# gabrielfnayres/new-vit

Hardware: AMD Instinct MI355X
Metric: volumes_per_sec_mst_dinov2_fwd (higher is better)
Workload: dtype bf16; 1 GPU; MST-DINOv2 (DinoV2ClassifierSlice, ViT-S/14) forward, 4 volumes/GPU of 64x512x512 bf16 zero-padded to 518x518 (N=1370 tokens/slice); global_batch_volumes=4, slices=64, parallelism=single GPU, weights=synthetic (mst.synth seed 2), random init of the reference architecture

## Files before the change

### new-vit_amd/csrc/k_gemm16_wreg.hip

```cpp
#include <cstdlib>

#include "mst_common.h"

namespace {

constexpr int KD = GEMM16_WREG_TILE.bk, BN = GEMM16_WREG_TILE.bn, CH = GEMM16_WREG_TILE.bm;
constexpr int ROWB = KD * 2;
constexpr int SLOT = CH * ROWB;
constexpr int WREG_NSLOT = 4;
constexpr int NSLOT = WREG_NSLOT;
constexpr int STG_PITCH = ROWB + 16;
constexpr int STG_BYTES = CH * STG_PITCH;
constexpr int STG_OFF = NSLOT * SLOT;
constexpr int LDS_BYTES = STG_OFF + 2 * STG_BYTES;
constexpr int NKT = KD / 32;
constexpr int PPW = SLOT / 1024 / 8;
static_assert(NSLOT == 4, "the counted vmcnt table below is written for three chunks in flight");

#define WREG_RD(dst, base, imm) asm volatile("ds_read_b128 %0, %1 offset:%2" : "=v"(dst) : "v"(base), "n"(imm) : "memory")

template <typename T, bool BLK>
__global__ __launch_bounds__(512) __attribute__((amdgpu_waves_per_eu(2, 2))) void gemm16_wreg_kernel(
    const T* __restrict__ A, int64_t lda, const T* __restrict__ W, int64_t ldw, const float* __restrict__ bias, T* __restrict__ C,
    int64_t ldc, int M, int N, float col_scale, int scale_cols, int nchunks) {
    typedef typename V8<T>::type vec8;
    typedef __attribute__((ext_vector_type(4))) T out4;
    extern __shared__ __attribute__((aligned(16))) char smem[];
    const int lane = threadIdx.x & 63;
    const int wave = __builtin_amdgcn_readfirstlane(threadIdx.x >> 6);
    const int frow = lane & 15, kq = lane >> 4;

    const int xcd = blockIdx.x & 7, g = blockIdx.x >> 3, G = gridDim.x >> 3;
    const int tiles_n = N / BN;
    const int nt = g % tiles_n, jcu = g / tiles_n;
    const int c_nt = (G - nt + tiles_n - 1) / tiles_n;
    const int per_xcd = (nchunks + 7) >> 3;
    const int lo = xcd * per_xcd;
    const int hi = lo + per_xcd < nchunks ? lo + per_xcd : nchunks;
    const int n0 = nt * BN + wave * 48;
    const float cs = nt * BN < scale_cols ? col_scale : 1.f;

    vec8 w[3][NKT];
#pragma unroll
    for (int t = 0; t < 3; ++t) {
        const T* wr = W + (int64_t)(n0 + 12 * (frow >> 2) + 4 * t + (frow & 3)) * ldw + kq * 8;
#pragma unroll
        for (int kt = 0; kt < NKT; ++kt) w[t][kt] = *reinterpret_cast<const vec8*>(wr + kt * 32);
    }
    f32x4 b[3];
#pragma unroll
    for (int t = 0; t < 3; ++t) {
        b[t] = (f32x4){0.f, 0.f, 0.f, 0.f};
        if (bias) b[t] = *reinterpret_cast<const f32x4*>(bias + n0 + 12 * kq + 4 * t);
    }
#pragma unroll
    for (int t = 0; t < 3; ++t) {
        asm volatile("" : "+v"(b[t]));
#pragma unroll
        for (int kt = 0; kt < NKT; ++kt) asm volatile("" : "+v"(w[t][kt]));
    }

    unsigned dma_off[PPW];
#pragma unroll
    for (int u = 0; u < PPW; ++u) {
        const int o = (wave * PPW + u) * 1024 + lane * 16;
        const int r = o / ROWB;
        dma_off[u] = BLK ? (unsigned)o : (unsigned)(r * (int)lda * 2 + ((((o % ROWB) >> 4) ^ (r & 15)) << 4));
    }
    const int64_t chunk_bytes = BLK ? (int64_t)SLOT : (int64_t)CH * lda * 2;
    auto issue_piece = [&](int chunk, int slot, int u) {
        const char* base = reinterpret_cast<const char*>(A) + (int64_t)chunk * chunk_bytes;
        unsigned off = dma_off[u];
        const int valid = M - chunk * CH;
        if (!BLK && valid < CH) {
            const int o = (wave * PPW + u) * 1024 + lane * 16;
            int r = o / ROWB;
            const int ck = ((o % ROWB) >> 4) ^ (r & 15);
            r = r < valid ? r : valid - 1;
            off = (unsigned)(r * (int)lda * 2 + ck * 16);
        }
        __builtin_amdgcn_global_load_lds(GLB_PTR(base + off), LDS_PTR(smem + slot * SLOT + (wave * PPW + u) * 1024), 16, 0, 0);
    };

    int rb[4];
#pragma unroll
    for (int j = 0; j < 4; ++j) rb[j] = BLK ? (kq >> 1) * 1024 + (frow + 32 * (kq & 1)) * 16 : frow * ROWB + (((4 * j + kq) ^ frow) << 4);
    const int put_off = frow * STG_PITCH + wave * 96 + kq * 24;
    int fl_lds[3];
    unsigned fl_glb[3];
    int fl_row[3];
#pragma unroll
    for (int j = 0; j < 3; ++j) {
        const int q = lane + 64 * j;
        fl_row[j] = wave * 4 + q / 48;
        fl_lds[j] = fl_row[j] * STG_PITCH + (q % 48) * 16;
        fl_glb[j] = (unsigned)(fl_row[j] * (int)ldc * 2 + nt * BN * 2 + (q % 48) * 16);
    }
    f32x4 acc[2][3];
    auto put = [&](int it) {
        char* stg = smem + STG_OFF + (it & 1) * STG_BYTES + put_off;
#pragma unroll
        for (int mt = 0; mt < 2; ++mt)
#pragma unroll
            for (int t = 0; t < 3; ++t) {
                out4 pk;
#pragma unroll
                for (int i = 0; i < 4; ++i) pk[i] = (T)(acc[mt][t][i] * cs);
                *reinterpret_cast<out4*>(stg + mt * 16 * STG_PITCH + t * 8) = pk;
            }
    };
    auto flush_piece = [&](int chunk, int it, int j) {
        const char* stg = smem + STG_OFF + (it & 1) * STG_BYTES;
        char* cb = reinterpret_cast<char*>(C) + (int64_t)chunk * CH * ldc * 2;
        const int valid = M - chunk * CH;
        const u32x4 v = *reinterpret_cast<const u32x4*>(stg + fl_lds[j]);
        if (valid >= CH || fl_row[j] < valid) {
            __builtin_nontemporal_store(v, reinterpret_cast<u32x4*>(cb + fl_glb[j]));
        }
    };
    auto flush = [&](int chunk, int it) {
#pragma unroll
        for (int j = 0; j < 3; ++j) flush_piece(chunk, it, j);
    };

    int c = lo + jcu;
    if (c >= hi) return;
#pragma unroll
    for (int d = 0; d < NSLOT - 1; ++d)
        if (c + d * c_nt < hi) {
#pragma unroll
            for (int u = 0; u < PPW; ++u) issue_piece(c + d * c_nt, d, u);
        }

    int prev = -1, last_it = 0;
    for (int it = 0; c < hi; c += c_nt, ++it) {
        if (c + 2 * c_nt < hi) {
            if (it <= 1) asm volatile("s_waitcnt vmcnt(6)" ::: "memory");
            else if (it == 2) asm volatile("s_waitcnt vmcnt(9)" ::: "memory");
            else asm volatile("s_waitcnt vmcnt(12)" ::: "memory");
        } else {
            asm volatile("s_waitcnt vmcnt(0)" ::: "memory");
        }
        asm volatile("s_waitcnt lgkmcnt(0)\n\ts_barrier" ::: "memory");
        if (prev >= 0) flush(prev, it - 1);

        const int slot = it % NSLOT;
        const int nxt = c + (NSLOT - 1) * c_nt, nslot = (it + NSLOT - 1) % NSLOT;
        const bool more = nxt < hi;
        int rbs[4];
#pragma unroll
        for (int j = 0; j < 4; ++j) rbs[j] = rb[j] + slot * SLOT;
#pragma unroll
        for (int mt = 0; mt < 2; ++mt)
#pragma unroll
            for (int t = 0; t < 3; ++t) acc[mt][t] = b[t];

        u32x4 a[2][2];
        WREG_RD(a[0][0], rbs[0], 0);
        if constexpr (BLK) WREG_RD(a[0][1], rbs[0], 256);
        else WREG_RD(a[0][1], rbs[0], 16 * ROWB);
#pragma unroll
        for (int kt = 0; kt < NKT; ++kt) {
            const int cur = kt & 1;
            if (kt + 1 < NKT) {
                switch (kt + 1) {
#define WREG_NEXT(KN)                                                                  \
    case KN:                                                                           \
        if constexpr (BLK) {                                                           \
            WREG_RD(a[(KN) & 1][0], rbs[0], (KN) * 2048);                              \
            WREG_RD(a[(KN) & 1][1], rbs[0], (KN) * 2048 + 256);                        \
        } else {                                                                       \
            WREG_RD(a[(KN) & 1][0], rbs[(KN) & 3], ((KN) >> 2) * 256);                 \
            WREG_RD(a[(KN) & 1][1], rbs[(KN) & 3], 16 * ROWB + ((KN) >> 2) * 256);     \
        }                                                                              \
        break;
                    WREG_NEXT(1) WREG_NEXT(2) WREG_NEXT(3) WREG_NEXT(4) WREG_NEXT(5) WREG_NEXT(6)
                    WREG_NEXT(7) WREG_NEXT(8) WREG_NEXT(9) WREG_NEXT(10) WREG_NEXT(11)
#undef WREG_NEXT
                }
                asm volatile("s_waitcnt lgkmcnt(2)" : "+v"(a[cur][0]), "+v"(a[cur][1])::"memory");
            } else {
                asm volatile("s_waitcnt lgkmcnt(0)" : "+v"(a[cur][0]), "+v"(a[cur][1])::"memory");
            }
            const vec8 a0 = __builtin_bit_cast(vec8, a[cur][0]), a1 = __builtin_bit_cast(vec8, a[cur][1]);
#pragma unroll
            for (int t = 0; t < 3; ++t) {
                acc[0][t] = mfma16(w[t][kt], a0, acc[0][t]);
                acc[1][t] = mfma16(w[t][kt], a1, acc[1][t]);
            }
            if ((kt & 3) == 1) {
                __builtin_amdgcn_sched_barrier(0);
                if (more) issue_piece(nxt, nslot, kt >> 2);
                __builtin_amdgcn_sched_barrier(0);
            }
        }
        put(it);
        prev = c;
        last_it = it;
    }
    asm volatile("s_waitcnt lgkmcnt(0)\n\ts_barrier" ::: "memory");
    flush(prev, last_it);
}

template <typename T, bool BLK>
int launch_t(const gemm_args& g) {
    static mst_lds_once lds_once;
    auto kern = gemm16_wreg_kernel<T, BLK>;
    mst_allow_lds((const void*)kern, LDS_BYTES, &lds_once);
    const int nchunks = (int)((g.M + CH - 1) / CH);
    kern<<<dim3(mst_persistent_grid()), dim3(512), LDS_BYTES, g.s>>>((const T*)g.A, g.lda, (const T*)g.W, g.ldw, g.bias, (T*)g.C, g.ldc, (int)g.M,
                                                                      g.N, g.col_scale, g.scale_cols, nchunks);
    return mst_check_launch("gemm16_wreg");
}

}

int launch_gemm16_wreg(const gemm_args& g, int a_blocked) {
    if (a_blocked) {
        if (g.dt == MST_BF16) return launch_t<bf16_t, true>(g);
        if (g.dt == MST_F16) return launch_t<f16_t, true>(g);
    }
    if (g.dt == MST_BF16) return launch_t<bf16_t, false>(g);
    if (g.dt == MST_F16) return launch_t<f16_t, false>(g);
    mst_set_error("gemm16_wreg: bad operand dtype %d", g.dt);
    return MST_EINVAL;
}
```

Baseline: 161.2 volumes/s.

## Balance QKV GEMM tiles across CUs and overlap epilogue with MFMA loop

Replaces the fixed tile-per-workgroup assignment with a segment schedule. Leftover column tiles that do not divide evenly across workgroups are split into short runs handled by spare workgroups, which reload weights for each segment. The schedule is checked at compile time for coverage and per-workgroup load bounds. The epilogue is now software-pipelined: the previous chunk's results are staged to LDS, and the chunk before that is read back and stored to global memory, interleaved between MFMA steps instead of in a serialized phase after the barrier. This aims to cut tail imbalance and epilogue stalls, at the cost of more complex waitcnt accounting and extra weight reloads for spare workgroups.

```diff
diff --git a/new-vit_amd/csrc/k_gemm16_wreg.hip b/new-vit_amd/csrc/k_gemm16_wreg.hip
--- a/new-vit_amd/csrc/k_gemm16_wreg.hip
+++ b/new-vit_amd/csrc/k_gemm16_wreg.hip
@@ -19,6 +19,53 @@
 
 #define WREG_RD(dst, base, imm) asm volatile("ds_read_b128 %0, %1 offset:%2" : "=v"(dst) : "v"(base), "n"(imm) : "memory")
 
+constexpr int WREG_RELOAD_UNITS = 2;
+constexpr int wreg_spare_run(int G, int T, int P) {
+    const int S = G % T;
+    if (!S) return 0;
+    int n = (2 * P + G) / (2 * G);
+    const int allow = ((T - 1) * WREG_RELOAD_UNITS + T - 1) / T;
+    n -= allow < n / 8 ? allow : n / 8;
+    if (S * n > P) n = P / S;
+    const int teams = G / T, bound = (T * P + G - 1) / G + 1;
+    while ((P - S * n + teams - 1) / teams > bound && T * (n + 1) <= bound) ++n;
+    return n;
+}
+struct wreg_seg { int tile, first, step, end; };
+constexpr int wreg_nseg(int g, int G, int T) { return g < G / T * T ? 1 : T; }
+constexpr wreg_seg wreg_segment(int g, int G, int T, int P, int k) {
+    const int teams = G / T, n = wreg_spare_run(G, T, P);
+    if (g < teams * T) return {g % T, (G % T) * n + g / T, teams, P};
+    const int s = g - teams * T;
+    return {k, s * n, 1, (s + 1) * n};
+}
+constexpr bool wreg_sched_ok(int G, int T, int P) {
+    int seen[4 * 1370] = {};
+    if (T * P > 4 * 1370 || T > G) return false;
+    const int bound = (T * P + G - 1) / G + 1;
+    for (int g = 0; g < G; ++g) {
+        int units = 0;
+        for (int k = 0; k < wreg_nseg(g, G, T); ++k) {
+            const wreg_seg s = wreg_segment(g, G, T, P, k);
+            if (s.tile < 0 || s.tile >= T || s.first < 0 || s.step < 1 || s.end > P) return false;
+            for (int c = s.first; c < s.end; c += s.step, ++units) ++seen[s.tile * P + c];
+        }
+        if (units > bound) return false;
+    }
+    for (int u = 0; u < T * P; ++u)
+        if (seen[u] != 1) return false;
+    return true;
+}
+constexpr bool wreg_sched_ok_all(int G) {
+    constexpr int Ps[] = {0, 1, 2, 3, 10, 11, 12, 33, 49, 1370};
+    for (int T = 1; T <= 4; ++T)
+        for (int P : Ps)
+            if (!wreg_sched_ok(G, T, P)) return false;
+    return true;
+}
+static_assert(wreg_sched_ok_all(32), "QKV schedule: a unit is missed or doubled, or a workgroup is over ceil(T P / G) + 1 (MI355X, 32 CUs per XCD)");
+static_assert(wreg_sched_ok_all(4) && wreg_sched_ok_all(5) && wreg_sched_ok_all(7), "QKV schedule at other CU counts per XCD");
+
 template <typename T, bool BLK>
 __global__ __launch_bounds__(512) __attribute__((amdgpu_waves_per_eu(2, 2))) void gemm16_wreg_kernel(
     const T* __restrict__ A, int64_t lda, const T* __restrict__ W, int64_t ldw, const float* __restrict__ bias, T* __restrict__ C,
@@ -32,33 +79,10 @@
 
     const int xcd = blockIdx.x & 7, g = blockIdx.x >> 3, G = gridDim.x >> 3;
     const int tiles_n = N / BN;
-    const int nt = g % tiles_n, jcu = g / tiles_n;
-    const int c_nt = (G - nt + tiles_n - 1) / tiles_n;
     const int per_xcd = (nchunks + 7) >> 3;
     const int lo = xcd * per_xcd;
-    const int hi = lo + per_xcd < nchunks ? lo + per_xcd : nchunks;
-    const int n0 = nt * BN + wave * 48;
-    const float cs = nt * BN < scale_cols ? col_scale : 1.f;
-
-    vec8 w[3][NKT];
-#pragma unroll
-    for (int t = 0; t < 3; ++t) {
-        const T* wr = W + (int64_t)(n0 + 12 * (frow >> 2) + 4 * t + (frow & 3)) * ldw + kq * 8;
-#pragma unroll
-        for (int kt = 0; kt < NKT; ++kt) w[t][kt] = *reinterpret_cast<const vec8*>(wr + kt * 32);
-    }
-    f32x4 b[3];
-#pragma unroll
-    for (int t = 0; t < 3; ++t) {
-        b[t] = (f32x4){0.f, 0.f, 0.f, 0.f};
-        if (bias) b[t] = *reinterpret_cast<const f32x4*>(bias + n0 + 12 * kq + 4 * t);
-    }
-#pragma unroll
-    for (int t = 0; t < 3; ++t) {
-        asm volatile("" : "+v"(b[t]));
-#pragma unroll
-        for (int kt = 0; kt < NKT; ++kt) asm volatile("" : "+v"(w[t][kt]));
-    }
+    const int P = lo >= nchunks ? 0 : lo + per_xcd < nchunks ? per_xcd : nchunks - lo;
+    const int nseg = wreg_nseg(g, G, tiles_n);
 
     unsigned dma_off[PPW];
 #pragma unroll
@@ -82,40 +106,58 @@
         __builtin_amdgcn_global_load_lds(GLB_PTR(base + off), LDS_PTR(smem + slot * SLOT + (wave * PPW + u) * 1024), 16, 0, 0);
     };
 
-    int rb[4];
-#pragma unroll
-    for (int j = 0; j < 4; ++j) rb[j] = BLK ? (kq >> 1) * 1024 + (frow + 32 * (kq & 1)) * 16 : frow * ROWB + (((4 * j + kq) ^ frow) << 4);
+    int rbs[4];
     const int put_off = frow * STG_PITCH + wave * 96 + kq * 24;
-    int fl_lds[3];
-    unsigned fl_glb[3];
-    int fl_row[3];
-#pragma unroll
-    for (int j = 0; j < 3; ++j) {
-        const int q = lane + 64 * j;
-        fl_row[j] = wave * 4 + q / 48;
-        fl_lds[j] = fl_row[j] * STG_PITCH + (q % 48) * 16;
-        fl_glb[j] = (unsigned)(fl_row[j] * (int)ldc * 2 + nt * BN * 2 + (q % 48) * 16);
-    }
+    auto fl_piece = [&](int j, int& row, int& col) {
+        int q = lane;
+        asm volatile("" : "+v"(q));
+        q += 64 * j;
+        const int r = (q >= 48) + (q >= 96) + (q >= 144);
+        row = wave * 4 + r;
+        col = q - 48 * r;
+    };
     f32x4 acc[2][3];
-    auto put = [&](int it) {
-        char* stg = smem + STG_OFF + (it & 1) * STG_BYTES + put_off;
+    vec8 w[3][NKT];
+    f32x4 b[3];
+    float cs = 1.f;
+    int nt = 0;
+    out4 pk[2][3];
+    auto pack = [&]() {
 #pragma unroll
         for (int mt = 0; mt < 2; ++mt)
 #pragma unroll
             for (int t = 0; t < 3; ++t) {
-                out4 pk;
-#pragma unroll
-                for (int i = 0; i < 4; ++i) pk[i] = (T)(acc[mt][t][i] * cs);
-                *reinterpret_cast<out4*>(stg + mt * 16 * STG_PITCH + t * 8) = pk;
+#pragma unroll
+                for (int i = 0; i < 4; ++i) pk[mt][t][i] = (T)(acc[mt][t][i] * cs);
+                acc[mt][t] = b[t];
             }
+    };
+    auto stage = [&](int it, int mt) {
+        char* stg = smem + STG_OFF + (it & 1) * STG_BYTES + put_off + mt * 16 * STG_PITCH;
+#pragma unroll
+        for (int t = 0; t < 3; ++t) *reinterpret_cast<out4*>(stg + t * 8) = pk[mt][t];
+    };
+    u32x4 fv;
+    auto flush_read = [&](int it, int j) {
+        int row, col;
+        fl_piece(j, row, col);
+        WREG_RD(fv, row * STG_PITCH + col * 16 + STG_OFF + (it & 1) * STG_BYTES, 0);
+    };
+    auto flush_store = [&](int chunk, int j) {
+        char* cb = reinterpret_cast<char*>(C) + (int64_t)chunk * CH * ldc * 2 + nt * BN * 2;
+        int row, col;
+        fl_piece(j, row, col);
+        __builtin_nontemporal_store(fv, reinterpret_cast<u32x4*>(cb + (unsigned)(row * (int)ldc * 2 + col * 16)));
     };
     auto flush_piece = [&](int chunk, int it, int j) {
         const char* stg = smem + STG_OFF + (it & 1) * STG_BYTES;
-        char* cb = reinterpret_cast<char*>(C) + (int64_t)chunk * CH * ldc * 2;
+        char* cb = reinterpret_cast<char*>(C) + (int64_t)chunk * CH * ldc * 2 + nt * BN * 2;
         const int valid = M - chunk * CH;
-        const u32x4 v = *reinterpret_cast<const u32x4*>(stg + fl_lds[j]);
-        if (valid >= CH || fl_row[j] < valid) {
-            __builtin_nontemporal_store(v, reinterpret_cast<u32x4*>(cb + fl_glb[j]));
+        int row, col;
+        fl_piece(j, row, col);
+        const u32x4 v = *reinterpret_cast<const u32x4*>(stg + row * STG_PITCH + col * 16);
+        if (valid >= CH || row < valid) {
+            __builtin_nontemporal_store(v, reinterpret_cast<u32x4*>(cb + (unsigned)(row * (int)ldc * 2 + col * 16)));
         }
     };
     auto flush = [&](int chunk, int it) {
@@ -123,83 +165,134 @@
         for (int j = 0; j < 3; ++j) flush_piece(chunk, it, j);
     };
 
-    int c = lo + jcu;
-    if (c >= hi) return;
-#pragma unroll
-    for (int d = 0; d < NSLOT - 1; ++d)
-        if (c + d * c_nt < hi) {
-#pragma unroll
-            for (int u = 0; u < PPW; ++u) issue_piece(c + d * c_nt, d, u);
-        }
-
-    int prev = -1, last_it = 0;
-    for (int it = 0; c < hi; c += c_nt, ++it) {
-        if (c + 2 * c_nt < hi) {
-            if (it <= 1) asm volatile("s_waitcnt vmcnt(6)" ::: "memory");
-            else if (it == 2) asm volatile("s_waitcnt vmcnt(9)" ::: "memory");
-            else asm volatile("s_waitcnt vmcnt(12)" ::: "memory");
-        } else {
-            asm volatile("s_waitcnt vmcnt(0)" ::: "memory");
+#pragma nounroll
+    for (int sg = 0; sg < nseg; ++sg) {
+        const wreg_seg seg = wreg_segment(g, G, tiles_n, P, sg);
+        int c = lo + seg.first;
+        const int hi = lo + seg.end, c_nt = seg.step;
+        if (c >= hi) continue;
+        nt = seg.tile;
+        cs = nt * BN < scale_cols ? col_scale : 1.f;
+        const int n0 = nt * BN + wave * 48;
+        int wl = lane;
+        asm volatile("" : "+v"(wl));
+        const int wrow = wl & 15, wkq = wl >> 4;
+#pragma unroll
+        for (int d = 0; d < NSLOT - 1; ++d)
+            if (c + d * c_nt < hi) {
+#pragma unroll
+                for (int u = 0; u < PPW; ++u) issue_piece(c + d * c_nt, d, u);
+            }
+
+#pragma unroll
+        for (int t = 0; t < 3; ++t) {
+            const T* wr = W + (int64_t)(n0 + 12 * (wrow >> 2) + 4 * t + (wrow & 3)) * ldw + wkq * 8;
+#pragma unroll
+            for (int kt = 0; kt < NKT; ++kt) w[t][kt] = *reinterpret_cast<const vec8*>(wr + kt * 32);
+        }
+#pragma unroll
+        for (int t = 0; t < 3; ++t) {
+            b[t] = (f32x4){0.f, 0.f, 0.f, 0.f};
+            if (bias) b[t] = *reinterpret_cast<const f32x4*>(bias + n0 + 12 * wkq + 4 * t);
+        }
+#pragma unroll
+        for (int t = 0; t < 3; ++t) {
+            asm volatile("" : "+v"(b[t]));
+#pragma unroll
+            for (int kt = 0; kt < NKT; ++kt) asm volatile("" : "+v"(w[t][kt]));
+        }
+
+#pragma unroll
+        for (int mt = 0; mt < 2; ++mt)
+#pragma unroll
+            for (int t = 0; t < 3; ++t) acc[mt][t] = b[t];
+#pragma unroll
+        for (int j = 0; j < 4; ++j) rbs[j] = BLK ? (wkq >> 1) * 1024 + (wrow + 32 * (wkq & 1)) * 16 : wrow * ROWB + (((4 * j + wkq) ^ wrow) << 4);
+        int prev = -1, last_it = 0;
+        for (int it = 0; c < hi; c += c_nt, ++it) {
+            if (c + 2 * c_nt < hi) {
+                if (it <= 2) asm volatile("s_waitcnt vmcnt(6)" ::: "memory");
+                else if (it == 3) asm volatile("s_waitcnt vmcnt(9)" ::: "memory");
+                else asm volatile("s_waitcnt vmcnt(12)" ::: "memory");
+            } else {
+                asm volatile("s_waitcnt vmcnt(0)" ::: "memory");
+            }
+            asm volatile("s_waitcnt lgkmcnt(0)\n\ts_barrier" ::: "memory");
+
+            const int slot = it % NSLOT;
+            const int nxt = c + (NSLOT - 1) * c_nt, nslot = (it + NSLOT - 1) % NSLOT;
+            const bool more = nxt < hi, staged = it >= 1, flushed = it >= 2;
+            const int old = c - 2 * c_nt;
+            asm volatile("" : "=v"(fv));
+
+            u32x4 a[2][2];
+            WREG_RD(a[0][0], rbs[0], 0);
+            if constexpr (BLK) WREG_RD(a[0][1], rbs[0], 256);
+            else WREG_RD(a[0][1], rbs[0], 16 * ROWB);
+#pragma unroll
+            for (int kt = 0; kt < NKT; ++kt) {
+                const int cur = kt & 1;
+                if (kt + 1 < NKT) {
+                    switch (kt + 1) {
+#define WREG_NEXT(KN)                                                                  \
+        case KN:                                                                           \
+            if constexpr (BLK) {                                                           \
+                WREG_RD(a[(KN) & 1][0], rbs[0], (KN) * 2048);                              \
+                WREG_RD(a[(KN) & 1][1], rbs[0], (KN) * 2048 + 256);                        \
+            } else {                                                                       \
+                WREG_RD(a[(KN) & 1][0], rbs[(KN) & 3], ((KN) >> 2) * 256);                 \
+                WREG_RD(a[(KN) & 1][1], rbs[(KN) & 3], 16 * ROWB + ((KN) >> 2) * 256);     \
+            }                                                                              \
+            break;
+                        WREG_NEXT(1) WREG_NEXT(2) WREG_NEXT(3) WREG_NEXT(4) WREG_NEXT(5) WREG_NEXT(6)
+                        WREG_NEXT(7) WREG_NEXT(8) WREG_NEXT(9) WREG_NEXT(10) WREG_NEXT(11)
+#undef WREG_NEXT
+                    }
+                    asm volatile("s_waitcnt lgkmcnt(2)" : "+v"(a[cur][0]), "+v"(a[cur][1])::"memory");
+                } else {
+                    asm volatile("s_waitcnt lgkmcnt(0)" : "+v"(a[cur][0]), "+v"(a[cur][1])::"memory");
+                }
+                const vec8 a0 = __builtin_bit_cast(vec8, a[cur][0]), a1 = __builtin_bit_cast(vec8, a[cur][1]);
+#pragma unroll
+                for (int t = 0; t < 3; ++t) {
+                    acc[0][t] = mfma16(w[t][kt], a0, acc[0][t]);
+                    acc[1][t] = mfma16(w[t][kt], a1, acc[1][t]);
+                }
+                if (kt == 0 || kt == 2) {
+                    __builtin_amdgcn_sched_barrier(0);
+                    if (staged) stage(it - 1, kt >> 1);
+                    __builtin_amdgcn_sched_barrier(0);
+                }
+                if ((kt & 3) == 1) {
+                    __builtin_amdgcn_sched_barrier(0);
+                    if (more) issue_piece(nxt, nslot, kt >> 2);
+                    __builtin_amdgcn_sched_barrier(0);
+                }
+                if (kt == 3 || kt == 5 || kt == 7) {
+                    __builtin_amdgcn_sched_barrier(0);
+                    if (flushed) flush_read(it, (kt - 3) >> 1);
+                    __builtin_amdgcn_sched_barrier(0);
+                }
+                if (kt == 4 || kt == 6 || kt == 8) {
+                    __builtin_amdgcn_sched_barrier(0);
+                    if (flushed) flush_store(old, (kt - 4) >> 1);
+                    __builtin_amdgcn_sched_barrier(0);
+                }
+            }
+            pack();
+            const int to_next = slot == NSLOT - 1 ? -(NSLOT - 1) * SLOT : SLOT;
+#pragma unroll
+            for (int j = 0; j < (BLK ? 1 : 4); ++j) rbs[j] += to_next;
+            prev = c;
+            last_it = it;
         }
         asm volatile("s_waitcnt lgkmcnt(0)\n\ts_barrier" ::: "memory");
-        if (prev >= 0) flush(prev, it - 1);
-
-        const int slot = it % NSLOT;
-        const int nxt = c + (NSLOT - 1) * c_nt, nslot = (it + NSLOT - 1) % NSLOT;
-        const bool more = nxt < hi;
-        int rbs[4];
-#pragma unroll
-        for (int j = 0; j < 4; ++j) rbs[j] = rb[j] + slot * SLOT;
-#pragma unroll
-        for (int mt = 0; mt < 2; ++mt)
-#pragma unroll
-            for (int t = 0; t < 3; ++t) acc[mt][t] = b[t];
-
-        u32x4 a[2][2];
-        WREG_RD(a[0][0], rbs[0], 0);
-        if constexpr (BLK) WREG_RD(a[0][1], rbs[0], 256);
-        else WREG_RD(a[0][1], rbs[0], 16 * ROWB);
-#pragma unroll
-        for (int kt = 0; kt < NKT; ++kt) {
-            const int cur = kt & 1;
-            if (kt + 1 < NKT) {
-                switch (kt + 1) {
-#define WREG_NEXT(KN)                                                                  \
-    case KN:                                                                           \
-        if constexpr (BLK) {                                                           \
-            WREG_RD(a[(KN) & 1][0], rbs[0], (KN) * 2048);                              \
-            WREG_RD(a[(KN) & 1][1], rbs[0], (KN) * 2048 + 256);                        \
-        } else {                                                                       \
-            WREG_RD(a[(KN) & 1][0], rbs[(KN) & 3], ((KN) >> 2) * 256);                 \
-            WREG_RD(a[(KN) & 1][1], rbs[(KN) & 3], 16 * ROWB + ((KN) >> 2) * 256);     \
-        }                                                                              \
-        break;
-                    WREG_NEXT(1) WREG_NEXT(2) WREG_NEXT(3) WREG_NEXT(4) WREG_NEXT(5) WREG_NEXT(6)
-                    WREG_NEXT(7) WREG_NEXT(8) WREG_NEXT(9) WREG_NEXT(10) WREG_NEXT(11)
-#undef WREG_NEXT
-                }
-                asm volatile("s_waitcnt lgkmcnt(2)" : "+v"(a[cur][0]), "+v"(a[cur][1])::"memory");
-            } else {
-                asm volatile("s_waitcnt lgkmcnt(0)" : "+v"(a[cur][0]), "+v"(a[cur][1])::"memory");
-            }
-            const vec8 a0 = __builtin_bit_cast(vec8, a[cur][0]), a1 = __builtin_bit_cast(vec8, a[cur][1]);
-#pragma unroll
-            for (int t = 0; t < 3; ++t) {
-                acc[0][t] = mfma16(w[t][kt], a0, acc[0][t]);
-                acc[1][t] = mfma16(w[t][kt], a1, acc[1][t]);
-            }
-            if ((kt & 3) == 1) {
-                __builtin_amdgcn_sched_barrier(0);
-                if (more) issue_piece(nxt, nslot, kt >> 2);
-                __builtin_amdgcn_sched_barrier(0);
-            }
-        }
-        put(it);
-        prev = c;
-        last_it = it;
+        stage(last_it, 0);
+        stage(last_it, 1);
+        if (last_it >= 1) flush(prev - c_nt, last_it - 1);
+        asm volatile("s_waitcnt lgkmcnt(0)\n\ts_barrier" ::: "memory");
+        flush(prev, last_it);
     }
-    asm volatile("s_waitcnt lgkmcnt(0)\n\ts_barrier" ::: "memory");
-    flush(prev, last_it);
 }
 
 template <typename T, bool BLK>
```

New measurement: 160.0 volumes/s. Within noise of the previous version (-0.7%).
